# wenxiaoshuai/Points-Matching

Hardware: AMD Instinct MI355X
Metric: descriptor-pair distances/s (BF-L2 2-NN + ratio stage); RANSAC hypotheses/s in `ransac` (higher is better)
Workload: dtype f32

## Files before the change

### points_matching_amd/csrc/filter_gather.hip

```cpp
#include "pm_common.hpp"

namespace {

constexpr int FG_ROWS = 256;
constexpr int FG_MAX_BLOCKS = 4096;
constexpr unsigned FG_SPIN_LIMIT = 200000u;

enum { FG_RATIO = 0, FG_MIDPOINT = 1, FG_CROSS = 2 };
struct FgCross {
    const pm_match* rev;
    int nt, kr, flags;
};
struct FgParam {
    float ratio;
    double cut;
    FgCross x;
};

template <int MODE>
__device__ __forceinline__ bool fg_keep(const pm_match* __restrict__ knn, int i, int k, const FgParam& prm, pm_match& best)
{
    const uint4 a = *reinterpret_cast<const uint4*>(knn + static_cast<size_t>(i) * k);
    best.queryIdx = static_cast<int>(a.x); best.trainIdx = static_cast<int>(a.y);
    best.imgIdx = static_cast<int>(a.z);   best.distance = __uint_as_float(a.w);
// ... 141 lines not shown
template <int MODE>
__global__ __launch_bounds__(FG_ROWS) void filter_ratio_gather(const pm_match* __restrict__ knn, int nq, int k,
                                                               float ratio, const float* __restrict__ kp1,
                                                               const float* __restrict__ kp2,
                                                               pm_match* __restrict__ good, float* __restrict__ xy1,
                                                               float* __restrict__ xy2, int* __restrict__ n_out,
                                                               unsigned* __restrict__ blk_counts, unsigned epoch,
                                                               const unsigned long long* __restrict__ mm,
                                                               double* __restrict__ minmax_out)
{
    fg_compact<MODE>(knn, nq, k, ratio, kp1, kp2, good, xy1, xy2, n_out, blk_counts, epoch, mm, minmax_out,
                     FgCross{nullptr, 0, 0, 0});
}

__global__ __launch_bounds__(FG_ROWS) void filter_cross_gather(const pm_match* __restrict__ knn, int nq, int k, float ratio,
                                                               const float* __restrict__ kp1, const float* __restrict__ kp2,
                                                               pm_match* __restrict__ good, float* __restrict__ xy1,
                                                               float* __restrict__ xy2, int* __restrict__ n_out,
                                                               unsigned* __restrict__ blk_counts, unsigned epoch, FgCross cross)
{
    fg_compact<FG_CROSS>(knn, nq, k, ratio, kp1, kp2, good, xy1, xy2, n_out, blk_counts, epoch, nullptr, nullptr, cross);
}

__global__ __launch_bounds__(256) void concat_points(const float* __restrict__ xy1_parts,
                                                     const float* __restrict__ xy2_parts,
                                                     const int* __restrict__ counts, int parts, int stride,
                                                     float* __restrict__ xy1, float* __restrict__ xy2,
                                                     int* __restrict__ n_out)
{
    const int p = blockIdx.y;
    int off = 0, total = 0;
    for (int r = 0; r < parts; ++r) {
        int c = counts[r];
        c = c < 0 ? 0 : (c > stride ? stride : c);
        if (r < p) off += c;
        total += c;
    }
    int cp = counts[p];
    cp = cp < 0 ? 0 : (cp > stride ? stride : cp);
    const int i = blockIdx.x * 256 + threadIdx.x;
    if (i < cp) {
        const size_t s = 2 * (static_cast<size_t>(p) * stride + i), d = 2 * static_cast<size_t>(off + i);
        xy1[d] = xy1_parts[s]; xy1[d + 1] = xy1_parts[s + 1];
        xy2[d] = xy2_parts[s]; xy2[d + 1] = xy2_parts[s + 1];
    }
    if (p == 0 && i == 0) *n_out = total;
// ... 22 lines not shown

}

extern "C" int pm_filter_ratio_gather_dev(pm_ctx* ctx, const pm_match* d_knn, int nq, int k, float ratio,
                                          const float* d_kp1_xy, const float* d_kp2_xy, pm_match* d_good,
                                          float* d_xy1, float* d_xy2, int32_t* d_n_good)
{
    PM_REQUIRE(ctx != nullptr && d_n_good != nullptr, PM_E_INVALID, "null argument");
    PM_REQUIRE(nq >= 0 && k >= 2, PM_E_INVALID, "ratio test needs k >= 2");
    PM_REQUIRE(nq == 0 || (d_knn && d_good), PM_E_INVALID, "null match buffers");
    PM_REQUIRE((d_kp1_xy == nullptr) == (d_kp2_xy == nullptr), PM_E_INVALID, "give both keypoint arrays or none");
    PM_REQUIRE(d_kp1_xy == nullptr || (d_xy1 && d_xy2), PM_E_INVALID, "null point outputs");
    PM_HIP_CHECK(hipSetDevice(ctx->device));
    pm::ScopedKernelTime t(ctx, "filter_gather");
    if (nq == 0) {
        PM_HIP_CHECK(hipMemsetAsync(d_n_good, 0, sizeof(int32_t), ctx->stream));
        return PM_OK;
    }
    int nblk = 0;
    const int rc = fg_prepare(ctx, nq, &nblk);
    if (rc != PM_OK) return rc;
    hipLaunchKernelGGL(filter_ratio_gather<FG_RATIO>, dim3(nblk), dim3(FG_ROWS), 0, ctx->stream, d_knn, nq, k, ratio,
                       d_kp1_xy, d_kp2_xy, d_good, d_xy1, d_xy2, d_n_good, ctx->fg_counts, ctx->fg_epoch, nullptr, nullptr);
    PM_HIP_CHECK(hipGetLastError());
    return PM_OK;
}

extern "C" int pm_filter_midpoint_gather_dev(pm_ctx* ctx, const pm_match* d_m, int n, int k, const float* d_kp1_xy,
                                             const float* d_kp2_xy, pm_match* d_good, float* d_xy1, float* d_xy2,
                                             int32_t* d_n_good, double* d_minmax)
{
    PM_REQUIRE(ctx != nullptr && d_n_good != nullptr, PM_E_INVALID, "null argument");
    PM_REQUIRE(n >= 0 && k >= 1, PM_E_INVALID, "need n >= 0, k >= 1");
    PM_REQUIRE(n == 0 || (d_m && d_good), PM_E_INVALID, "null match buffers");
    PM_REQUIRE((d_kp1_xy == nullptr) == (d_kp2_xy == nullptr), PM_E_INVALID, "give both keypoint arrays or none");
    PM_REQUIRE(d_kp1_xy == nullptr || (d_xy1 && d_xy2), PM_E_INVALID, "null point outputs");
    PM_HIP_CHECK(hipSetDevice(ctx->device));
    pm::ScopedKernelTime t(ctx, "filter_gather");
    if (n == 0) {
        PM_HIP_CHECK(hipMemsetAsync(d_n_good, 0, sizeof(int32_t), ctx->stream));
        if (d_minmax) {
            const double init[2] = {1.0, 0.0};
            PM_HIP_CHECK(hipMemcpyAsync(d_minmax, init, sizeof init, hipMemcpyHostToDevice, ctx->stream));
            PM_HIP_CHECK(hipStreamSynchronize(ctx->stream));
        }
        return PM_OK;
// ... 58 lines not shown
```

### points_matching_amd/csrc/knn_constants.hpp

```cpp
#pragma once

namespace pm_knn {

constexpr int KNN_C = 4;
constexpr int QB = 128;
constexpr int TT32 = 64;
constexpr float KNN_BIG = 3.0e38f;

constexpr int H_DP = 128;
constexpr int H_ROW = H_DP + 16;
constexpr int H_LDS_ROW = H_ROW + 8;
constexpr int H_NCH = H_ROW / 16;
constexpr int H_TT = 128;
constexpr int H_QB = 256;
constexpr float H_MAXABS = 361.f;
constexpr int H_ROW16 = H_ROW / 8;
constexpr int H_LDS_ROW16 = H_LDS_ROW / 8;

constexpr int I8_BITS = 256;
constexpr int I8_NCH = 8;
constexpr int I8_ROW16 = 16;
constexpr int I8_LDS_ROW16 = 17;
constexpr int I8_GROUP_ROWS = 8;
constexpr int I8_SHIFT = 16;
constexpr int I8_EMPTY = static_cast<int>(0x80000000u);
constexpr int I8W_BITS = 512;
constexpr int I8W_NCH = 16;
constexpr int I8W_ROW16 = 32;

constexpr int U8_DP = 128;
constexpr int U8_NCH = 4;
constexpr int U8_ROW16 = 8;
constexpr int U8_LDS_ROW16 = 9;
constexpr int U8_SHIFT = 9;
constexpr int U8_PAD_SEED = -(1 << 22);
constexpr int U8_WIDE_ROW16 = 9;
constexpr int F16S_NCH = 8;
constexpr int F16S_ROW16 = 16;
constexpr int F16S_LDS_ROW16 = 17;
constexpr int SEED_TILE_BYTES = H_TT * 4;

}
```

### points_matching_amd/csrc/knn_l2.hip

```cpp
#include <cstdlib>

#include "knn_l2_plan.hpp"
#include "knn_shared.hpp"

namespace {

using namespace pm_knn;

constexpr int TILE_T = 64;
constexpr int PM_U8_FUSED_MAX_NQ = 768;
__host__ inline bool u8_fused_by_default(int nq) { return nq <= PM_U8_FUSED_MAX_NQ; }
constexpr float KNN_INF = __builtin_inff();

__device__ __forceinline__ uint32_t f32_bits(float f) { return __float_as_uint(f); }

__device__ __forceinline__ uint64_t knn_key(float dist, int idx)
{
    uint32_t b = (dist != dist) ? 0x7FC00000u : f32_bits(dist);
    return (static_cast<uint64_t>(b) << 32) | static_cast<uint32_t>(idx);
}

template <bool VEC4>
__device__ __forceinline__ float l2sqr_canonical(const float* __restrict__ a,
                                                 const float* __restrict__ b, int dim)
// ... 677 lines not shown
        const float t = a[j] - b[j];
        const float p = t * t;
        d = d + p;
    }
    return d;
}

struct KnnFuse {
    float ratio;
    const float* kp1;
    const float* kp2;
    pm_match* good;
    float* xy1;
    float* xy2;
    int* n_out;
    unsigned long long* pk;
    unsigned long long* tile;
    unsigned* tilecnt;
    unsigned* err;
    unsigned epoch;
};
constexpr int KF_TILE_BLOCKS = 8;
constexpr unsigned KF_SPIN_LIMIT = 1u << 22;

template <bool VEC4, int NS, bool FUSE, bool GEN, int KM>
__global__ __launch_bounds__(256) __attribute__((amdgpu_num_sgpr(80))) void knn_l2_refine(
    const float* __restrict__ Q, const float* __restrict__ T, const float* __restrict__ qnorm,
    const unsigned long long* __restrict__ stats, unsigned epoch, unsigned* __restrict__ diag, int nq, int nt,
    int dim, int k, KnnGeom g16, KnnGeom g32, int route, pm_match* __restrict__ out, KnnFuse fz)
{
    __shared__ int clist[4][64 * NS];
    const int lane = threadIdx.x & 63, wave = threadIdx.x >> 6;
    int q = __builtin_amdgcn_readfirstlane(blockIdx.x * 4 + wave);
    bool ghost = false;
    if (q >= nq) {
        if (!FUSE) return;
        ghost = true;
        q = nq - 1;
    }
    const float* qp = Q + static_cast<size_t>(q) * dim;
    const float na = qnorm[q];
    const unsigned long long s0 = stats[0], s1 = stats[1];
    const float tmax = static_cast<unsigned>(s0 >> 32) == epoch ? __uint_as_float(static_cast<unsigned>(s0)) : 0.f;
    const bool flagged = static_cast<unsigned>(s1 >> 32) == epoch;
    const bool ineligible = flagged && (s1 & 2ull);
    bool general = false;
    if constexpr (GEN) {
        const unsigned long long s3 = stats[3];
        const bool gen_off = static_cast<unsigned>(s3 >> 32) == epoch;
        general = route == ROUTE_AUTO && ineligible && !gen_off;
    }
    const bool hinted = route == ROUTE_F16_HINT || route == ROUTE_U8_HINT;
    const bool use16 = hinted || (route == ROUTE_AUTO && (!ineligible || general));
    const bool nonfinite = (flagged && (s1 & 1ull)) || (hinted && ineligible);
    const KnnGeom g = use16 ? g16 : g32;
    float unscale = 1.f, eps_c = g.eps_coef, eps_abs = 0.f;
    bool unranked = false;
    if constexpr (GEN) {
        if (general) {
// ... 98 lines not shown
    } else {
        for (int j = lane; j < nt; j += 64) {
            const float d =
                __builtin_sqrtf(l2sqr_canonical<VEC4>(qp, T + static_cast<size_t>(j) * dim, dim));
            b.insert(knn_key(d, j), d);
        }
    }
    int nn_idx[2] = {-1, -1};
    float nn_d[2] = {KNN_INF, KNN_INF};
    for (int c = 0; c < k; ++c) {
        const uint64_t best = wave_min_u64(b.k[0]);
        const unsigned long long owners = __ballot(b.k[0] == best);
        const int first = __ffsll(static_cast<long long>(owners)) - 1;
        const float dist = __shfl(b.d[0], first, 64);
        if (lane == first) b.pop();
        pm_match m;
        m.queryIdx = q;
        m.imgIdx = 0;
        if (best == ~0ull) { m.trainIdx = -1; m.distance = KNN_INF; }
        else { m.trainIdx = static_cast<int>(static_cast<uint32_t>(best)); m.distance = dist; }
        if (c < 2) { nn_idx[c] = m.trainIdx; nn_d[c] = m.distance; }
        if (lane == 0 && !ghost && out) out[static_cast<size_t>(q) * k + c] = m;
    }
    if (!FUSE) return;

    __shared__ unsigned s_keep[4];
    __shared__ unsigned s_bits;
    __shared__ int s_last;
    __shared__ int s_pre[4];
    const int tid = threadIdx.x;
    {
        const float rhs = fz.ratio * nn_d[1];
        const bool keep = !ghost && nn_idx[0] >= 0 && nn_idx[1] >= 0 && nn_d[0] < rhs;
        if (lane == 0) {
            if (!ghost)
                __hip_atomic_store(&fz.pk[q], (static_cast<unsigned long long>(f32_bits(nn_d[0])) << 32) |
                                                  static_cast<unsigned long long>(static_cast<uint32_t>(nn_idx[0])),
                                   __ATOMIC_RELAXED, __HIP_MEMORY_SCOPE_AGENT);
            s_keep[wave] = keep ? 1u : 0u;
        }
    }
    asm volatile("s_waitcnt vmcnt(0)" ::: "memory");
    __syncthreads();
    const int blk = static_cast<int>(blockIdx.x), tile = blk / KF_TILE_BLOCKS;
    const int nblk = static_cast<int>(gridDim.x), ntiles = (nblk + KF_TILE_BLOCKS - 1) / KF_TILE_BLOCKS;
    if (tid == 0) {
// ... 104 lines not shown
#pragma unroll
                for (int i = 0; i < U8_ROW16 / 2; ++i) tv[i] = tp[hf * (U8_ROW16 / 2) + i];
#pragma unroll
                for (int i = 0; i < U8_ROW16 / 2; ++i) {
                    const uint4 a = qv[hf * (U8_ROW16 / 2) + i];
                    acc = __builtin_amdgcn_sdot4(static_cast<int>(a.x), static_cast<int>(tv[i].x), acc, false);
                    acc = __builtin_amdgcn_sdot4(static_cast<int>(a.y), static_cast<int>(tv[i].y), acc, false);
                    acc = __builtin_amdgcn_sdot4(static_cast<int>(a.z), static_cast<int>(tv[i].z), acc, false);
                    acc = __builtin_amdgcn_sdot4(static_cast<int>(a.w), static_cast<int>(tv[i].w), acc, false);
                }
                asm volatile("" : "+v"(acc));
            }
            d2[u] = qn + static_cast<int>(tnorm[ok[u] ? row : row_begin]) - 2 * acc;
        }
#pragma unroll
        for (int u = 0; u < U; ++u) {
            const int row = base + u * LANES + me;
            const float d = __builtin_sqrtf(static_cast<float>(d2[u]));
            if (ok[u]) tb.insert(knn_key(d, row), d);
        }
    }
}

template <int NS, int GROUP, int KM, bool FUSE>
__global__ __launch_bounds__(256) void knn_l2_refine8(
    const float* __restrict__ Q, const float* __restrict__ T, const uint4* __restrict__ Q8, const uint4* __restrict__ T8,
    const float* __restrict__ qnorm, const float* __restrict__ tnorm, const int* __restrict__ cand,
    const unsigned long long* __restrict__ stats, unsigned epoch, unsigned* __restrict__ diag, int nq, int nt, int dim, int k,
    int slots, int tiles_per_split, pm_match* __restrict__ out, KnnFuse fz, int t_row16)
{
    constexpr int GPB = 16 / GROUP;
    constexpr int IMAX = 0x7FFFFFFF;
    __shared__ int clist[4][4][16 * NS];
    const int lane = threadIdx.x & 63, wave = threadIdx.x >> 6;
    const int qi = lane >> 4, l = lane & 15;
    const int q = blockIdx.x * 16 + wave * 4 + qi;
    const bool live = q < nq;
    const int qc = live ? q : nq - 1;
    const unsigned long long s1 = stats[1];
    const bool wrong_hint = static_cast<unsigned>(s1 >> 32) == epoch;
    if (diag && threadIdx.x == 0 && blockIdx.x == 0) diag[2] = 3u;
    const int qn = static_cast<int>(qnorm[qc]);
    const int* cv = cand + static_cast<size_t>(qc) * slots;
    uint4 qv[U8_ROW16];
#pragma unroll
    for (int i = 0; i < U8_ROW16; ++i) qv[i] = Q8[static_cast<size_t>(qc) * U8_ROW16 + i];

    int val[NS], code[NS];
    MinN<int, KM> mn;
    mn.init(IMAX);
#pragma unroll
    for (int i = 0; i < NS; ++i) {
        const int s = l + 16 * i;
// ... 97 lines not shown
            }
            for (int j = 0; j < KM; ++j) {
                const uint64_t m = pm::wave_min_u64(tb.k[0]);
                if (tb.k[0] == m && m != ~0ull) tb.pop();
                if (lane == src && m != ~0ull) b.insert(m, __uint_as_float(static_cast<unsigned>(m >> 32)));
            }
        }
    }
    int nn_idx[2] = {-1, -1};
    float nn_d[2] = {KNN_INF, KNN_INF};
    for (int c = 0; c < k; ++c) {
        const uint64_t best = row_min_u64(b.k[0]);
        const unsigned owners = static_cast<unsigned>(__ballot(b.k[0] == best) >> (16 * qi)) & 0xFFFFu;
        const int first = __ffs(static_cast<int>(owners)) - 1;
        const float dist = __shfl(b.d[0], 16 * qi + first, 64);
        if (l == first) b.pop();
        pm_match m;
        m.queryIdx = q;
        m.imgIdx = 0;
        if (best == ~0ull) { m.trainIdx = -1; m.distance = KNN_INF; }
        else { m.trainIdx = static_cast<int>(static_cast<uint32_t>(best)); m.distance = dist; }
        if (c < 2) { nn_idx[c] = m.trainIdx; nn_d[c] = m.distance; }
        if (l == 0 && live && out) out[static_cast<size_t>(q) * k + c] = m;
    }
    if constexpr (FUSE) {
        __shared__ unsigned s_bits[4];
        __shared__ unsigned long long s_rec[16];
        __shared__ int s_pre[4];
        const int tid = threadIdx.x;
        const float rhs = fz.ratio * nn_d[1];
        const bool keep = live && nn_idx[0] >= 0 && nn_idx[1] >= 0 && nn_d[0] < rhs;
        if (l == 0)
            s_rec[wave * 4 + qi] = (static_cast<unsigned long long>(f32_bits(nn_d[0])) << 32) |
                                   static_cast<unsigned long long>(static_cast<uint32_t>(nn_idx[0]));
        const unsigned long long bal = __ballot(l == 0 && keep);
        if (lane == 0)
            s_bits[wave] = static_cast<unsigned>(bal & 1ull) | (static_cast<unsigned>((bal >> 16) & 1ull) << 1) |
                           (static_cast<unsigned>((bal >> 32) & 1ull) << 2) | (static_cast<unsigned>((bal >> 48) & 1ull) << 3);
        __syncthreads();
        const unsigned bits = s_bits[0] | (s_bits[1] << 4) | (s_bits[2] << 8) | (s_bits[3] << 12);
        const int cnt = __popc(bits);
        const int blk = static_cast<int>(blockIdx.x);
        if (tid == 0)
            __hip_atomic_store(&fz.tilecnt[blk], (fz.epoch << 8) | static_cast<unsigned>(cnt), __ATOMIC_RELAXED, __HIP_MEMORY_SCOPE_AGENT);
        int before = 0;
        for (int j = tid; j < blk; j += 256) {
// ... 235 lines not shown
    const int tiles = (nq + queries_per_tile - 1) / queries_per_tile;
    if (tiles > ctx->kf_cap) {
        PM_HIP_CHECK(hipStreamSynchronize(ctx->stream));
        if (ctx->kf_tile) PM_HIP_CHECK(hipFree(ctx->kf_tile));
        ctx->kf_tile = nullptr;
        ctx->kf_cap = 0;
        const int cap = tiles < 4096 ? 4096 : tiles + tiles / 2;
        PM_HIP_CHECK(hipMalloc(reinterpret_cast<void**>(&ctx->kf_tile), static_cast<size_t>(cap) * 12));
        PM_HIP_CHECK(hipMemsetAsync(ctx->kf_tile, 0, static_cast<size_t>(cap) * 12, ctx->stream));
        ctx->kf_cap = cap;
        ctx->kf_epoch = 0;
    }
    if (++ctx->kf_epoch >= (1u << 24)) {
        PM_HIP_CHECK(hipMemsetAsync(ctx->kf_tile, 0, static_cast<size_t>(ctx->kf_cap) * 12, ctx->stream));
        ctx->kf_epoch = 1;
    }
    fz.tile = ctx->kf_tile;
    fz.tilecnt = reinterpret_cast<unsigned*>(ctx->kf_tile + ctx->kf_cap);
    fz.err = reinterpret_cast<unsigned*>(ctx->knn_stats) + 12;
    fz.epoch = ctx->kf_epoch;
    return PM_OK;
}

KnnL2Request knn_l2_request(const pm_ctx* ctx, const void* q, const void* t, bool u8_rows, int nq, int nt, int dim, int k, int flags,
                            bool fuse)
{
    KnnL2Request r{};
    r.nq = nq; r.nt = nt; r.dim = dim; r.k = k; r.flags = flags; r.n_cu = ctx->n_cu;
    std::memcpy(r.opts, ctx->opts, sizeof(r.opts));
    r.u8_rows = u8_rows;
    r.aligned = ((reinterpret_cast<uintptr_t>(q) | reinterpret_cast<uintptr_t>(t)) & (u8_rows ? 3 : 15)) == 0;
    r.fuse = fuse;
    return r;
}

KnnGeom knn_geom(const KnnGeomPlan& g, const float* cand)
{
    return KnnGeom{cand, g.slots, g.tiles_per_split, g.rows_per_tile, g.lid_mask, g.eps_coef, g.embed_coef, g.eps_coef_gen,
                   g.abs_gen, g.int_shift};
}

int knn_l2_enqueue(pm_ctx* ctx, const KnnL2Plan& p, const float* dq, int nq, const float* dt, int nt, int dim, int k,
                   pm_match* dout, const KnnFuse* fuse, const uint8_t* uq = nullptr, const uint8_t* ut = nullptr)
{
    PM_REFUSE_CAPTURE(ctx);
    int rc = pm::arena_reserve(ctx, p.need);
    if (rc != PM_OK) return rc;
    pm::arena_reset(ctx);
    float* qnorm = static_cast<float*>(pm::arena_take(ctx, p.qnorm_bytes));
    float* tnorm = static_cast<float*>(pm::arena_take(ctx, p.tnorm_bytes));
    float* cval32 = p.want32 ? static_cast<float*>(pm::arena_take(ctx, p.c32)) : nullptr;
    float* cval16 = p.want16 ? static_cast<float*>(pm::arena_take(ctx, p.c16)) : nullptr;
    _Float16* Qh = p.want16 ? static_cast<_Float16*>(pm::arena_take(ctx, p.qh)) : nullptr;
    _Float16* Th = p.want16 ? static_cast<_Float16*>(pm::arena_take(ctx, p.th)) : nullptr;
    void* seeds = p.sdb ? pm::arena_take(ctx, p.sdb) : nullptr;
    void* Qf = p.qfb ? pm::arena_take(ctx, p.qfb) : nullptr;
    PM_REQUIRE(qnorm && tnorm && (!p.want32 || cval32) && (!p.want16 || (cval16 && Qh && Th)) && (!p.sdb || seeds) && (!p.qfb || Qf),
               PM_E_NOMEM, "scratch arena too small");
    KnnFuse fz{};
    if (fuse) {
        fz = *fuse;
        fz.pk = static_cast<unsigned long long*>(pm::arena_take(ctx, p.pkb));
        PM_REQUIRE(fz.pk != nullptr, PM_E_NOMEM, "scratch arena too small");
        rc = kf_prepare(ctx, nq, fz, p.kf_tile);
        if (rc != PM_OK) return rc;
    }
    const KnnGeom g32 = knn_geom(p.g32, cval32), g16 = knn_geom(p.g16, cval16);

    unsigned long long* stats = ctx->knn_stats;
    if (++ctx->knn_epoch == 0u) {
        PM_HIP_CHECK(hipMemsetAsync(stats, 0, 32, ctx->stream));
        ctx->knn_epoch = 1u;
    }
    const unsigned epoch = ctx->knn_epoch;
    unsigned* diag = nullptr;
    if (ctx->knn_diag) {
        diag = ctx->knn_diag_words;
        PM_HIP_CHECK(hipMemsetAsync(diag, 0, 12, ctx->stream));
    }
    const int nq_pad = p.nq_pad, nt_pad = p.nt_pad, t_wide = p.t_wide, route = p.route;
    {
        pm::ScopedKernelTime t(ctx, "knn_l2_prep");
        const dim3 grid(p.prep_grid);
#define PM_PREP_DP_AL(LAUNCH_)                                                                                            \
    do {                                                                                                                  \
        if (p.dp16 == 128) { if (p.vec) LAUNCH_(128, true); else LAUNCH_(128, false); }                                   \
        else { if (p.vec) LAUNCH_(256, true); else LAUNCH_(256, false); }                                                 \
    } while (0)
#define PM_PREP16U(DP_, AL_)                                                                                              \
// ... 39 lines not shown
#undef PM_PREP_DP_AL
        PM_HIP_CHECK(hipGetLastError());
    }
    if (route == ROUTE_U8_HINT) {
        rc = launch_coarse_u8(ctx, Qh, Qf, Th, static_cast<const int*>(seeds), nq, nq_pad, nt, p.splits16, g16.tiles_per_split,
                              reinterpret_cast<int*>(cval16), g16.slots, p.u8_group, p.u8_form);
        if (rc != PM_OK) return rc;
    } else if (p.f16s) {
        rc = launch_coarse_f16s(ctx, Qh, Th, static_cast<const float*>(seeds), nq, nq_pad, nt, p.splits16, g16.tiles_per_split,
                                ~g16.lid_mask, cval16, g16.slots);
        if (rc != PM_OK) return rc;
    } else if (p.want16) {
        rc = launch_coarse_f16(ctx, Qh, Th, nq, nq_pad, nt, p.splits16, g16.tiles_per_split, ~g16.lid_mask, cval16,
                               g16.slots, stats, epoch, route == ROUTE_AUTO ? 1 : 0, p.dp16);
        if (rc != PM_OK) return rc;
    }
    if (p.want32) {
        rc = launch_coarse_f32(ctx, dq, nq, dt, nt, dim, tnorm, p.splits32, g32.tiles_per_split, ~g32.lid_mask, cval32,
                               g32.slots, stats, epoch, route == ROUTE_AUTO ? 1 : 0);
        if (rc != PM_OK) return rc;
    }
    pm::ScopedKernelTime t(ctx, "knn_l2_refine");
    if (p.refine8) {
#define PM_R8K(NS_, GROUP_, KM_, FUSE_)                                                                                    \
    hipLaunchKernelGGL((knn_l2_refine8<NS_, GROUP_, KM_, FUSE_>), dim3((nq + 15) / 16), dim3(256), 0, ctx->stream, dq, dt,  \
                       reinterpret_cast<const uint4*>(Qh), reinterpret_cast<const uint4*>(Th), qnorm, tnorm,               \
                       reinterpret_cast<const int*>(cval16), stats, epoch, diag, nq, nt, dim, k, g16.slots, g16.tiles_per_split, dout, fz, \
                       t_wide ? U8_WIDE_ROW16 : U8_ROW16)
#define PM_R8(NS_, GROUP_) do { if (p.refine_fuse) PM_R8K(NS_, GROUP_, 2, true); else if (p.refine_km == 2) PM_R8K(NS_, GROUP_, 2, false); else PM_R8K(NS_, GROUP_, 4, false); } while (0)
#define PM_R8G(NS_) do { if (p.refine_group == 4) PM_R8(NS_, 4); else if (p.refine_group == 8) PM_R8(NS_, 8); else PM_R8(NS_, 16); } while (0)
        switch (p.refine_ns) {
        case 1: PM_R8G(1); break;
        case 2: PM_R8G(2); break;
        case 4: PM_R8G(4); break;
        case 8: PM_R8G(8); break;
        default: PM_R8G(16); break;
        }
#undef PM_R8G
#undef PM_R8
#undef PM_R8K
    } else {
#define PM_REFINE5(VEC_, NS_, FUSE_, GEN_, KM_)                                                                      \
    hipLaunchKernelGGL((knn_l2_refine<VEC_, NS_, FUSE_, GEN_, KM_>), dim3((nq + 3) / 4), dim3(256), 0, ctx->stream, dq, dt,  \
                       qnorm, stats, epoch, diag, nq, nt, dim, k, g16, g32, route, dout, fz)
#define PM_REFINE4(VEC_, NS_, FUSE_, GEN_) do { if (p.refine_km == 2) PM_REFINE5(VEC_, NS_, FUSE_, GEN_, 2); else PM_REFINE5(VEC_, NS_, false, GEN_, 4); } while (0)
#define PM_REFINE3(NS_, FUSE_, GEN_) do { if (p.refine_vec) PM_REFINE4(true, NS_, FUSE_, GEN_); else PM_REFINE4(false, NS_, FUSE_, GEN_); } while (0)
#define PM_REFINE2(NS_, FUSE_) do { if (p.refine_gen) PM_REFINE3(NS_, FUSE_, true); else PM_REFINE3(NS_, FUSE_, false); } while (0)
#define PM_REFINE(NS_) do { if (p.refine_fuse) PM_REFINE2(NS_, true); else PM_REFINE2(NS_, false); } while (0)
        switch (p.refine_ns) {
        case 1: PM_REFINE(1); break;
        case 2: PM_REFINE(2); break;
        case 4: PM_REFINE(4); break;
        default: PM_REFINE(8); break;
        }
#undef PM_REFINE5
#undef PM_REFINE4
#undef PM_REFINE3
#undef PM_REFINE2
#undef PM_REFINE
    }
    PM_HIP_CHECK(hipGetLastError());
    return PM_OK;
}

int knn_l2_run(pm_ctx* ctx, const float* dq, int nq, const float* dt, int nt, int dim, int k, int flags, pm_match* dout,
               const KnnFuse* fuse, int* verdict, const uint8_t* uq = nullptr, const uint8_t* ut = nullptr)
{
    const bool u8 = uq != nullptr;
    const KnnL2Plan p = knn_l2_plan(knn_l2_request(ctx, u8 ? static_cast<const void*>(uq) : dq, u8 ? static_cast<const void*>(ut) : dt, u8,
                                                   nq, nt, dim, k, flags, fuse != nullptr));
    *verdict = p.verdict;
    if (p.verdict == KNN_EXACT) return run_exact(ctx, dq, nq, dt, nt, dim, k, dout);
    if (p.verdict == KNN_WIDEN) return PM_OK;
    return knn_l2_enqueue(ctx, p, dq, nq, dt, nt, dim, k, dout, fuse, uq, ut);
}

}

extern "C" int pm_bf_knn_l2_f32_dev(pm_ctx* ctx, const float* dq, int nq, const float* dt, int nt, int dim,
                                    int k, int flags, pm_match* dout)
{
    PM_REQUIRE(ctx != nullptr, PM_E_INVALID, "ctx is null");
    PM_REQUIRE(nq >= 0 && nt >= 0 && dim >= 1 && k >= 1 && k <= PM_MAX_K, PM_E_INVALID,
               "need nq,nt >= 0, dim >= 1, 1 <= k <= PM_MAX_K");
    PM_REQUIRE(nq == 0 || (dq && dout), PM_E_INVALID, "null query/output pointer");
    PM_REQUIRE(nt == 0 || dt, PM_E_INVALID, "null train pointer");
    if (nq == 0) return PM_OK;
    PM_HIP_CHECK(hipSetDevice(ctx->device));
    PM_REFUSE_CAPTURE(ctx);
    int verdict;
    return knn_l2_run(ctx, dq, nq, dt, nt, dim, k, flags, dout, nullptr, &verdict);
}

extern "C" int pm_bf_knn_l2_ratio_dev(pm_ctx* ctx, const float* d_q, int nq, const float* d_t, int nt, int dim, int flags,
                                      float ratio, const float* d_kp1_xy, const float* d_kp2_xy, pm_match* d_knn,
                                      pm_match* d_good, float* d_xy1, float* d_xy2, int32_t* d_n_good)
{
// ... 1 lines not shown
    PM_REQUIRE(nq >= 0 && nt >= 0 && dim >= 1, PM_E_INVALID, "need nq,nt >= 0, dim >= 1");
    PM_REQUIRE(nq == 0 || (d_q && d_good), PM_E_INVALID, "null query/output pointer");
    PM_REQUIRE(nt == 0 || d_t, PM_E_INVALID, "null train pointer");
    PM_REQUIRE((d_kp1_xy == nullptr) == (d_kp2_xy == nullptr), PM_E_INVALID, "give both keypoint arrays or none");
    PM_REQUIRE(d_kp1_xy == nullptr || (d_xy1 && d_xy2), PM_E_INVALID, "null point outputs");
    PM_HIP_CHECK(hipSetDevice(ctx->device));
    PM_REFUSE_CAPTURE(ctx);
    if (nq == 0) {
        PM_HIP_CHECK(hipMemsetAsync(d_n_good, 0, sizeof(int32_t), ctx->stream));
        return PM_OK;
    }
    KnnFuse fz{};
    fz.ratio = ratio; fz.kp1 = d_kp1_xy; fz.kp2 = d_kp2_xy; fz.good = d_good; fz.xy1 = d_xy1; fz.xy2 = d_xy2; fz.n_out = d_n_good;
    const int fusion = ctx->opts[PM_OPT_FILTER_FUSION];
    const bool u8_hint = (flags & PM_KNN_HINT_U8) && !(flags & (PM_KNN_FORCE_F32 | PM_KNN_FORCE_EXACT));
    const bool separate = fusion == 1 || (fusion == 0 && d_knn != nullptr && !(u8_hint && u8_fused_by_default(nq)));
    int rc, verdict;
    if (!separate) {
        rc = knn_l2_run(ctx, d_q, nq, d_t, nt, dim, 2, flags, d_knn, &fz, &verdict);
        if (rc != PM_OK || verdict == KNN_MATRIX) return rc;
        return pm_filter_ratio_gather_dev(ctx, d_knn, nq, 2, ratio, d_kp1_xy, d_kp2_xy, d_good, d_xy1, d_xy2, d_n_good);
    }
    PM_REQUIRE(d_knn != nullptr, PM_E_INVALID, "the two-launch form needs d_knn");
    rc = knn_l2_run(ctx, d_q, nq, d_t, nt, dim, 2, flags, d_knn, nullptr, &verdict);
    if (rc != PM_OK) return rc;
    return pm_filter_ratio_gather_dev(ctx, d_knn, nq, 2, ratio, d_kp1_xy, d_kp2_xy, d_good, d_xy1, d_xy2, d_n_good);
}

namespace {
int u8_widened(pm_ctx* ctx, const uint8_t* dq, int nq, const uint8_t* dt, int nt, int dim, const float** fq, const float** ft)
{
    const size_t a = pm::align_up(static_cast<size_t>(nq) * dim, 64), b = static_cast<size_t>(nt) * dim;
    if ((a + b) * sizeof(float) > ctx->widen_cap) {
        PM_HIP_CHECK(hipStreamSynchronize(ctx->stream));
        if (ctx->widen) PM_HIP_CHECK(hipFree(ctx->widen));
        ctx->widen = nullptr;
        ctx->widen_cap = 0;
        const size_t cap = pm::align_up((a + b) * sizeof(float) * 5 / 4, size_t(1) << 20);
        PM_HIP_CHECK(hipMalloc(reinterpret_cast<void**>(&ctx->widen), cap));
        ctx->widen_cap = cap;
    }
    if (static_cast<size_t>(nq) * dim)
        hipLaunchKernelGGL(knn_u8_widen, dim3(256), dim3(256), 0, ctx->stream, dq, static_cast<size_t>(nq) * dim, ctx->widen);
    if (b) hipLaunchKernelGGL(knn_u8_widen, dim3(256), dim3(256), 0, ctx->stream, dt, b, ctx->widen + a);
    PM_HIP_CHECK(hipGetLastError());
    *fq = ctx->widen;
    *ft = ctx->widen + a;
    return PM_OK;
// ... 22 lines not shown

extern "C" int pm_bf_knn_l2_u8_ratio_dev(pm_ctx* ctx, const uint8_t* d_q, int nq, const uint8_t* d_t, int nt, int dim, float ratio,
                                         const float* d_kp1_xy, const float* d_kp2_xy, pm_match* d_knn, pm_match* d_good,
                                         float* d_xy1, float* d_xy2, int32_t* d_n_good)
{
    PM_REQUIRE(ctx != nullptr && d_n_good != nullptr && d_knn != nullptr, PM_E_INVALID, "null argument (the u8 form needs the record buffer)");
    PM_REQUIRE(nq >= 0 && nt >= 0 && dim >= 1, PM_E_INVALID, "need nq,nt >= 0, dim >= 1");
    PM_REQUIRE(nq == 0 || (d_q && d_good), PM_E_INVALID, "null query/output pointer");
    PM_REQUIRE((d_kp1_xy == nullptr) == (d_kp2_xy == nullptr), PM_E_INVALID, "give both keypoint arrays or none");
    PM_REQUIRE(d_kp1_xy == nullptr || (d_xy1 && d_xy2), PM_E_INVALID, "null point outputs");
    PM_HIP_CHECK(hipSetDevice(ctx->device));
    PM_REFUSE_CAPTURE(ctx);
    if (nq == 0) {
        PM_HIP_CHECK(hipMemsetAsync(d_n_good, 0, sizeof(int32_t), ctx->stream));
        return PM_OK;
    }
    const int fusion = ctx->opts[PM_OPT_FILTER_FUSION];
    if (fusion == 2 || (fusion == 0 && u8_fused_by_default(nq))) {
        KnnFuse fz{};
        fz.ratio = ratio; fz.kp1 = d_kp1_xy; fz.kp2 = d_kp2_xy; fz.good = d_good; fz.xy1 = d_xy1; fz.xy2 = d_xy2; fz.n_out = d_n_good;
        int verdict;
        const int rf = knn_l2_run(ctx, nullptr, nq, nullptr, nt, dim, 2, 0, d_knn, &fz, &verdict, d_q, d_t);
        if (rf != PM_OK || verdict != KNN_WIDEN) return rf;
    }
    const int rc = pm_bf_knn_l2_u8_dev(ctx, d_q, nq, d_t, nt, dim, 2, d_knn);
    if (rc != PM_OK) return rc;
    return pm_filter_ratio_gather_dev(ctx, d_knn, nq, 2, ratio, d_kp1_xy, d_kp2_xy, d_good, d_xy1, d_xy2, d_n_good);
}

extern "C" int pm_bf_knn_l2_u8(pm_ctx* ctx, const uint8_t* q, int nq, const uint8_t* t, int nt, int dim, int k, pm_match* out)
{
    PM_REQUIRE(ctx != nullptr, PM_E_INVALID, "ctx is null");
    PM_REQUIRE(nq >= 0 && nt >= 0 && dim >= 1 && k >= 1 && k <= PM_MAX_K, PM_E_INVALID,
               "need nq,nt >= 0, dim >= 1, 1 <= k <= PM_MAX_K");
    PM_REQUIRE(nq == 0 || (q && out), PM_E_INVALID, "null query/output pointer");
    PM_REQUIRE(nt == 0 || t, PM_E_INVALID, "null train pointer");
    if (nq == 0) return PM_OK;
    PM_HIP_CHECK(hipSetDevice(ctx->device));
    return pm::StagedBlock::knn(ctx, __func__, q, static_cast<size_t>(nq) * dim, t, static_cast<size_t>(nt) * dim, out,
                                  sizeof(pm_match) * static_cast<size_t>(nq) * k, [&](void* dq, void* dt, void* dout) {
        return pm_bf_knn_l2_u8_dev(ctx, static_cast<const uint8_t*>(dq), nq, static_cast<const uint8_t*>(dt), nt, dim, k,
                                   static_cast<pm_match*>(dout));
    });
}

extern "C" int pm_bf_knn_l2_f32(pm_ctx* ctx, const float* q, int nq, const float* t, int nt, int dim, int k,
// ... 16 lines not shown
```

### points_matching_amd/csrc/pm_capi.cpp

```cpp
#include <cfloat>
#include <cmath>

#include "pm_common.hpp"

namespace pm {

static thread_local char g_err[512] = "";

void set_error(const char* fmt, ...)
{
    va_list ap;
    va_start(ap, fmt);
    vsnprintf(g_err, sizeof g_err, fmt, ap);
    va_end(ap);
}

int arena_reserve(pm_ctx* ctx, size_t bytes)
{
    if (bytes <= ctx->arena_cap) return PM_OK;
    PM_HIP_CHECK(hipStreamSynchronize(ctx->stream));
    if (ctx->arena) PM_HIP_CHECK(hipFree(ctx->arena));
    ctx->arena = nullptr;
    ctx->arena_cap = 0;
    size_t cap = align_up(bytes + bytes / 4, size_t(1) << 20);
// ... 154 lines not shown
    if (e != hipSuccess) {
        set_error("hipMalloc failed: %s", hipGetErrorString(e));
        (void)hipStreamDestroy(c->own_stream);
        delete c;
        return PM_E_NOMEM;
    }
    c->knn_diag_words = reinterpret_cast<unsigned*>(c->knn_stats + 4);
    *out = c;
    return PM_OK;
}

int pm_ctx_destroy(pm_ctx* ctx)
{
    if (!ctx) return PM_OK;
    (void)hipSetDevice(ctx->device);
    (void)hipStreamSynchronize(ctx->stream);
    drain_timers(ctx);
    for (hipEvent_t e : ctx->event_pool) (void)hipEventDestroy(e);
    if (ctx->arena) (void)hipFree(ctx->arena);
    if (ctx->knn_stats) (void)hipFree(ctx->knn_stats);
    if (ctx->fg_counts) (void)hipFree(ctx->fg_counts);
    if (ctx->sync_words) (void)hipFree(ctx->sync_words);
    if (ctx->kf_tile) (void)hipFree(ctx->kf_tile);
    if (ctx->widen) (void)hipFree(ctx->widen);
    if (ctx->feat) (void)hipFree(ctx->feat);
    if (ctx->desc_tab) (void)hipFree(ctx->desc_tab);
    if (ctx->pinned) (void)hipHostFree(ctx->pinned);
    if (ctx->own_stream) (void)hipStreamDestroy(ctx->own_stream);
    delete ctx;
    return PM_OK;
}

int pm_ctx_set_stream(pm_ctx* ctx, void* hip_stream)
{
    PM_REQUIRE(ctx != nullptr, PM_E_INVALID, "ctx is null");
    PM_HIP_CHECK(hipStreamSynchronize(ctx->stream));
    ctx->stream = hip_stream ? static_cast<hipStream_t>(hip_stream) : ctx->own_stream;
    return PM_OK;
}

int pm_ctx_synchronize(pm_ctx* ctx)
{
    PM_REQUIRE(ctx != nullptr, PM_E_INVALID, "ctx is null");
    PM_HIP_CHECK(hipStreamSynchronize(ctx->stream));
    return PM_OK;
}
// ... 330 lines not shown
```

### points_matching_amd/csrc/pm_common.hpp

```cpp
#pragma once
#include <hip/hip_runtime.h>

#include <cstdarg>
#include <cstdint>
#include <cstdio>
#include <cstring>
#include <map>
#include <string>
#include <vector>

#include "pm.h"
#include "stage_layout.hpp"

namespace pm {

void set_error(const char* fmt, ...);

#define PM_HIP_CHECK(expr)                                                              \
    do {                                                                                \
        hipError_t e_ = (expr);                                                         \
        if (e_ != hipSuccess) {                                                         \
            ::pm::set_error("%s failed: %s (%s:%d)", #expr, hipGetErrorString(e_),      \
                            __FILE__, __LINE__);                                        \
            return PM_E_HIP;                                                            \
// ... 29 lines not shown

struct pm_ctx {
    int device = 0;
    hipStream_t own_stream = nullptr;
    hipStream_t stream = nullptr;
    char* arena = nullptr;
    size_t arena_cap = 0;
    size_t arena_off = 0;
    void* pinned = nullptr;
    size_t pinned_cap = 0;
    bool timing = false;
    std::map<std::string, pm::KernelTimer> timers;
    std::vector<hipEvent_t> event_pool;
    int n_cu = 256;
    unsigned long long* knn_stats = nullptr;
    unsigned* knn_diag_words = nullptr;
    unsigned knn_epoch = 0;
    bool knn_diag = false;
    unsigned* fg_counts = nullptr;
    unsigned fg_epoch = 0;
    unsigned long long* kf_tile = nullptr;
    int kf_cap = 0;
    unsigned kf_epoch = 0;
    int* sync_words = nullptr;
    int opts[PM_OPT_COUNT_] = {};
    float* widen = nullptr;
    size_t widen_cap = 0;
    char* feat = nullptr;
    size_t feat_cap = 0;
    size_t feat_counter_off = 0;
    int feat_noct = 0;
    int feat_w[16] = {}, feat_h[16] = {};
    size_t feat_off[16] = {};
    char* desc_tab = nullptr;
};

namespace pm {

int arena_reserve(pm_ctx* ctx, size_t bytes);
void arena_reset(pm_ctx* ctx);
void* arena_take(pm_ctx* ctx, size_t bytes);
int pinned_reserve(pm_ctx* ctx, size_t bytes);
struct __attribute__((visibility("hidden"))) StagedBlock : StageLayout {
    pm_ctx* ctx;
    const char* who;
    char* base = nullptr;
    int rc = PM_OK;
    StagedBlock(pm_ctx* c, const char* w) : ctx(c), who(w) {}
    StagedBlock(const StagedBlock&) = delete;
    ~StagedBlock();
    int alloc();
    void upload(size_t off, const void* src, size_t bytes);
    void download(void* dst, size_t off, size_t bytes);
    int sync();
    template <class T> T* at(size_t off) const { return reinterpret_cast<T*>(base + off); }
    void step(hipError_t e, int status, const char* what);
    template <class Dev> static int knn(pm_ctx* ctx, const char* who, const void* q, size_t qb, const void* t, size_t tb, void* out, size_t ob, Dev dev)
    {
        StagedBlock bq(ctx, who), bt(ctx, who), bo(ctx, who);
        const size_t o_q = bq.add(qb), o_t = bt.add(tb), o_out = bo.add(ob);
        if (bq.alloc() != PM_OK || bt.alloc() != PM_OK || bo.alloc() != PM_OK) return PM_E_NOMEM;
        bq.upload(o_q, q, qb);
        if (bq.rc == PM_OK) bt.upload(o_t, t, tb);
        if (bq.rc != PM_OK || bt.rc != PM_OK) return PM_E_HIP;
        bo.rc = dev(bq.base, bt.base, bo.base);
// ... 58 lines not shown
```

Measured before the change: 2272 billion.

## Emit ratio-test keep masks from refine kernel and compact via mask prefix sums

In the two-launch, non-fused k=2 path, the refine kernel now evaluates the ratio test itself and writes one keep bit per query into a small mask buffer. A new compaction kernel reads those masks and computes global offsets by having each block popcount all preceding mask words. This replaces the ratio-filter kernel's cross-block counter handshake with spin waits and its re-evaluation of the test. The cost is a redundant O(blocks²) popcount over mask words, a new device mask buffer, and an extra template variant for the refine kernels.

```diff
diff --git a/points_matching_amd/csrc/filter_gather.hip b/points_matching_amd/csrc/filter_gather.hip
--- a/points_matching_amd/csrc/filter_gather.hip
+++ b/points_matching_amd/csrc/filter_gather.hip
@@ -1,3 +1,4 @@
+#include "knn_constants.hpp"
 #include "pm_common.hpp"
 
 namespace {
@@ -187,6 +188,60 @@
     fg_compact<FG_CROSS>(knn, nq, k, ratio, kp1, kp2, good, xy1, xy2, n_out, blk_counts, epoch, nullptr, nullptr, cross);
 }
 
+__global__ __launch_bounds__(FG_ROWS) void filter_masks_kernel(const uint4* __restrict__ masks, const pm_match* __restrict__ knn,
+                                                               int nq, int k, const float* __restrict__ kp1,
+                                                               const float* __restrict__ kp2, pm_match* __restrict__ good,
+                                                               float* __restrict__ xy1, float* __restrict__ xy2,
+                                                               int* __restrict__ n_out)
+{
+    __shared__ int wave_cnt[FG_ROWS / 64];
+    __shared__ int wave_pre[FG_ROWS / 64];
+    const int tid = threadIdx.x, lane = tid & 63, wave = tid >> 6;
+    const int b = blockIdx.x;
+    const int i = b * FG_ROWS + tid;
+    constexpr int V16 = FG_ROWS / 64;
+    const int ic = i < nq ? i : nq - 1;
+    const uint4 a = *reinterpret_cast<const uint4*>(knn + static_cast<size_t>(ic) * k);
+    const uint4 own = masks[b * V16 + wave];
+    float2 pa = {0.f, 0.f}, pb = {0.f, 0.f};
+    if (kp1) pa = *reinterpret_cast<const float2*>(kp1 + 2 * static_cast<size_t>(ic));
+    int before = 0;
+    for (int v = tid; v < b * V16; v += FG_ROWS) {
+        const uint4 m = masks[v];
+        before += __popc(m.x) + __popc(m.y) + __popc(m.z) + __popc(m.w);
+    }
+    if (kp1) {
+        const int tr = static_cast<int>(a.y);
+        pb = *reinterpret_cast<const float2*>(kp2 + 2 * static_cast<size_t>(tr >= 0 ? tr : 0));
+    }
+    const unsigned ow = (lane >> 4) == 0 ? own.x : (lane >> 4) == 1 ? own.y : (lane >> 4) == 2 ? own.z : own.w;
+    const bool keep = i < nq && ((ow >> (8 * ((lane >> 2) & 3) + (lane & 3))) & 1u);
+#pragma unroll
+    for (int o = 32; o > 0; o >>= 1) before += __shfl_xor(before, o, 64);
+    const unsigned long long bal = __ballot(keep);
+    if (lane == 0) { wave_cnt[wave] = __popcll(bal); wave_pre[wave] = before; }
+    __syncthreads();
+    int off = __popcll(bal & ((1ull << lane) - 1ull));
+    int tot = 0;
+#pragma unroll
+    for (int w = 0; w < FG_ROWS / 64; ++w) {
+        off += wave_pre[w];
+        if (w < wave) off += wave_cnt[w];
+        tot += wave_pre[w] + wave_cnt[w];
+    }
+    if (keep) {
+        pm_match best;
+        best.queryIdx = static_cast<int>(a.x); best.trainIdx = static_cast<int>(a.y);
+        best.imgIdx = static_cast<int>(a.z);   best.distance = __uint_as_float(a.w);
+        good[off] = best;
+        if (kp1) {
+            *reinterpret_cast<float2*>(xy1 + 2 * static_cast<size_t>(off)) = pa;
+            *reinterpret_cast<float2*>(xy2 + 2 * static_cast<size_t>(off)) = pb;
+        }
+    }
+    if (b == static_cast<int>(gridDim.x) - 1 && tid == 0) *n_out = tot;
+}
+
 __global__ __launch_bounds__(256) void concat_points(const float* __restrict__ xy1_parts,
                                                      const float* __restrict__ xy2_parts,
                                                      const int* __restrict__ counts, int parts, int stride,
@@ -255,6 +310,22 @@
     if (rc != PM_OK) return rc;
     hipLaunchKernelGGL(filter_ratio_gather<FG_RATIO>, dim3(nblk), dim3(FG_ROWS), 0, ctx->stream, d_knn, nq, k, ratio,
                        d_kp1_xy, d_kp2_xy, d_good, d_xy1, d_xy2, d_n_good, ctx->fg_counts, ctx->fg_epoch, nullptr, nullptr);
+    PM_HIP_CHECK(hipGetLastError());
+    return PM_OK;
+}
+
+static_assert(FG_ROWS == pm_knn::KM_BLOCK_ROWS && FG_MAX_BLOCKS * FG_ROWS == pm_knn::KM_MAX_ROWS,
+              "the mask buffer is sized in this compaction's blocks");
+
+int pm::filter_masks_gather(pm_ctx* ctx, const pm_match* d_knn, int nq, int k, const float* d_kp1_xy, const float* d_kp2_xy,
+                            pm_match* d_good, float* d_xy1, float* d_xy2, int32_t* d_n_good)
+{
+    const int nblk = (nq + FG_ROWS - 1) / FG_ROWS;
+    PM_REQUIRE(nq >= 1 && nblk <= FG_MAX_BLOCKS, PM_E_UNSUPPORTED, "more than 1M query rows per compaction call");
+    PM_REQUIRE(ctx->km_masks != nullptr && pm_knn::knn_mask_bytes(nq) <= ctx->km_cap, PM_E_INVALID, "no keep masks for this many rows");
+    pm::ScopedKernelTime t(ctx, "filter_gather");
+    hipLaunchKernelGGL(filter_masks_kernel, dim3(nblk), dim3(FG_ROWS), 0, ctx->stream, reinterpret_cast<const uint4*>(ctx->km_masks),
+                       d_knn, nq, k, d_kp1_xy, d_kp2_xy, d_good, d_xy1, d_xy2, d_n_good);
     PM_HIP_CHECK(hipGetLastError());
     return PM_OK;
 }
diff --git a/points_matching_amd/csrc/knn_constants.hpp b/points_matching_amd/csrc/knn_constants.hpp
--- a/points_matching_amd/csrc/knn_constants.hpp
+++ b/points_matching_amd/csrc/knn_constants.hpp
@@ -1,4 +1,5 @@
 #pragma once
+#include <cstddef>
 
 namespace pm_knn {
 
@@ -40,4 +41,17 @@
 constexpr int F16S_LDS_ROW16 = 17;
 constexpr int SEED_TILE_BYTES = H_TT * 4;
 
+constexpr int KM_BLOCK_ROWS = 256;
+constexpr int KM_BLOCK_BYTES = KM_BLOCK_ROWS / 4;
+constexpr int KM_MAX_ROWS = 4096 * KM_BLOCK_ROWS;
+inline size_t knn_mask_bytes(int nq)
+{
+    return (static_cast<size_t>(nq) + KM_BLOCK_ROWS - 1) / KM_BLOCK_ROWS * KM_BLOCK_BYTES;
 }
+inline size_t knn_mask_capacity(size_t need)
+{
+    const size_t want = need + need / 2;
+    return want < 4096 ? 4096 : (want + KM_BLOCK_BYTES - 1) / KM_BLOCK_BYTES * KM_BLOCK_BYTES;
+}
+
+}
diff --git a/points_matching_amd/csrc/knn_l2.hip b/points_matching_amd/csrc/knn_l2.hip
--- a/points_matching_amd/csrc/knn_l2.hip
+++ b/points_matching_amd/csrc/knn_l2.hip
@@ -723,19 +723,21 @@
 };
 constexpr int KF_TILE_BLOCKS = 8;
 constexpr unsigned KF_SPIN_LIMIT = 1u << 22;
-
-template <bool VEC4, int NS, bool FUSE, bool GEN, int KM>
+enum { KNN_TAIL_NONE = 0, KNN_TAIL_FUSE = 1, KNN_TAIL_MASK = 2 };
+
+template <bool VEC4, int NS, int TAIL, bool GEN, int KM>
 __global__ __launch_bounds__(256) __attribute__((amdgpu_num_sgpr(80))) void knn_l2_refine(
     const float* __restrict__ Q, const float* __restrict__ T, const float* __restrict__ qnorm,
     const unsigned long long* __restrict__ stats, unsigned epoch, unsigned* __restrict__ diag, int nq, int nt,
-    int dim, int k, KnnGeom g16, KnnGeom g32, int route, pm_match* __restrict__ out, KnnFuse fz)
-{
+    int dim, int k, KnnGeom g16, KnnGeom g32, int route, pm_match* __restrict__ out, KnnFuse fz, uint8_t* __restrict__ masks)
+{
+    constexpr bool FUSE = TAIL == KNN_TAIL_FUSE;
     __shared__ int clist[4][64 * NS];
     const int lane = threadIdx.x & 63, wave = threadIdx.x >> 6;
     int q = __builtin_amdgcn_readfirstlane(blockIdx.x * 4 + wave);
     bool ghost = false;
     if (q >= nq) {
-        if (!FUSE) return;
+        if (TAIL == KNN_TAIL_NONE) return;
         ghost = true;
         q = nq - 1;
     }
@@ -880,6 +882,14 @@
         if (c < 2) { nn_idx[c] = m.trainIdx; nn_d[c] = m.distance; }
         if (lane == 0 && !ghost && out) out[static_cast<size_t>(q) * k + c] = m;
     }
+    if constexpr (TAIL == KNN_TAIL_MASK) {
+        __shared__ unsigned s_bit[4];
+        const float rhs = fz.ratio * nn_d[1];
+        const bool keep = !ghost && nn_idx[0] >= 0 && nn_idx[1] >= 0 && nn_d[0] < rhs;
+        if (lane == 0) s_bit[wave] = keep ? 1u << wave : 0u;
+        __syncthreads();
+        if (threadIdx.x == 0) masks[blockIdx.x] = static_cast<uint8_t>(s_bit[0] | s_bit[1] | s_bit[2] | s_bit[3]);
+    }
     if (!FUSE) return;
 
     __shared__ unsigned s_keep[4];
@@ -1030,13 +1040,14 @@
     }
 }
 
-template <int NS, int GROUP, int KM, bool FUSE>
+template <int NS, int GROUP, int KM, int TAIL>
 __global__ __launch_bounds__(256) void knn_l2_refine8(
     const float* __restrict__ Q, const float* __restrict__ T, const uint4* __restrict__ Q8, const uint4* __restrict__ T8,
     const float* __restrict__ qnorm, const float* __restrict__ tnorm, const int* __restrict__ cand,
     const unsigned long long* __restrict__ stats, unsigned epoch, unsigned* __restrict__ diag, int nq, int nt, int dim, int k,
-    int slots, int tiles_per_split, pm_match* __restrict__ out, KnnFuse fz, int t_row16)
-{
+    int slots, int tiles_per_split, pm_match* __restrict__ out, KnnFuse fz, uint8_t* __restrict__ masks, int t_row16)
+{
+    constexpr bool FUSE = TAIL == KNN_TAIL_FUSE;
     constexpr int GPB = 16 / GROUP;
     constexpr int IMAX = 0x7FFFFFFF;
     __shared__ int clist[4][4][16 * NS];
@@ -1180,6 +1191,14 @@
         else { m.trainIdx = static_cast<int>(static_cast<uint32_t>(best)); m.distance = dist; }
         if (c < 2) { nn_idx[c] = m.trainIdx; nn_d[c] = m.distance; }
         if (l == 0 && live && out) out[static_cast<size_t>(q) * k + c] = m;
+    }
+    if constexpr (TAIL == KNN_TAIL_MASK) {
+        const float rhs = fz.ratio * nn_d[1];
+        const bool keep = live && nn_idx[0] >= 0 && nn_idx[1] >= 0 && nn_d[0] < rhs;
+        const unsigned long long bal = __ballot(l == 0 && keep);
+        if (lane == 0)
+            masks[blockIdx.x * 4 + wave] = static_cast<uint8_t>((bal & 1ull) | (((bal >> 16) & 1ull) << 1) |
+                                                                (((bal >> 32) & 1ull) << 2) | (((bal >> 48) & 1ull) << 3));
     }
     if constexpr (FUSE) {
         __shared__ unsigned s_bits[4];
@@ -1461,6 +1480,21 @@
     return PM_OK;
 }
 
+int km_prepare(pm_ctx* ctx, int nq)
+{
+    const size_t need = knn_mask_bytes(nq);
+    if (need > ctx->km_cap) {
+        PM_HIP_CHECK(hipStreamSynchronize(ctx->stream));
+        if (ctx->km_masks) PM_HIP_CHECK(hipFree(ctx->km_masks));
+        ctx->km_masks = nullptr;
+        ctx->km_cap = 0;
+        const size_t cap = knn_mask_capacity(need);
+        PM_HIP_CHECK(hipMalloc(reinterpret_cast<void**>(&ctx->km_masks), cap));
+        ctx->km_cap = cap;
+    }
+    return PM_OK;
+}
+
 KnnL2Request knn_l2_request(const pm_ctx* ctx, const void* q, const void* t, bool u8_rows, int nq, int nt, int dim, int k, int flags,
                             bool fuse)
 {
@@ -1480,7 +1514,8 @@
 }
 
 int knn_l2_enqueue(pm_ctx* ctx, const KnnL2Plan& p, const float* dq, int nq, const float* dt, int nt, int dim, int k,
-                   pm_match* dout, const KnnFuse* fuse, const uint8_t* uq = nullptr, const uint8_t* ut = nullptr)
+                   pm_match* dout, const KnnFuse* fuse, const uint8_t* uq = nullptr, const uint8_t* ut = nullptr,
+                   const float* mask_ratio = nullptr)
 {
     PM_REFUSE_CAPTURE(ctx);
     int rc = pm::arena_reserve(ctx, p.need);
@@ -1504,6 +1539,14 @@
         rc = kf_prepare(ctx, nq, fz, p.kf_tile);
         if (rc != PM_OK) return rc;
     }
+    const bool mask_tail = mask_ratio != nullptr && !p.refine_fuse && p.refine_km == 2;
+    PM_REQUIRE(mask_ratio == nullptr || mask_tail, PM_E_INVALID, "the mask tail needs a k = 2 plan without the fused tail");
+    if (mask_tail) {
+        fz.ratio = *mask_ratio;
+        rc = km_prepare(ctx, nq);
+        if (rc != PM_OK) return rc;
+    }
+    uint8_t* masks = mask_tail ? ctx->km_masks : nullptr;
     const KnnGeom g32 = knn_geom(p.g32, cval32), g16 = knn_geom(p.g16, cval16);
 
     unsigned long long* stats = ctx->knn_stats;
@@ -1589,12 +1632,12 @@
     }
     pm::ScopedKernelTime t(ctx, "knn_l2_refine");
     if (p.refine8) {
-#define PM_R8K(NS_, GROUP_, KM_, FUSE_)                                                                                    \
-    hipLaunchKernelGGL((knn_l2_refine8<NS_, GROUP_, KM_, FUSE_>), dim3((nq + 15) / 16), dim3(256), 0, ctx->stream, dq, dt,  \
+#define PM_R8K(NS_, GROUP_, KM_, TAIL_)                                                                                    \
+    hipLaunchKernelGGL((knn_l2_refine8<NS_, GROUP_, KM_, TAIL_>), dim3((nq + 15) / 16), dim3(256), 0, ctx->stream, dq, dt,  \
                        reinterpret_cast<const uint4*>(Qh), reinterpret_cast<const uint4*>(Th), qnorm, tnorm,               \
                        reinterpret_cast<const int*>(cval16), stats, epoch, diag, nq, nt, dim, k, g16.slots, g16.tiles_per_split, dout, fz, \
-                       t_wide ? U8_WIDE_ROW16 : U8_ROW16)
-#define PM_R8(NS_, GROUP_) do { if (p.refine_fuse) PM_R8K(NS_, GROUP_, 2, true); else if (p.refine_km == 2) PM_R8K(NS_, GROUP_, 2, false); else PM_R8K(NS_, GROUP_, 4, false); } while (0)
+                       masks, t_wide ? U8_WIDE_ROW16 : U8_ROW16)
+#define PM_R8(NS_, GROUP_) do { if (p.refine_fuse) PM_R8K(NS_, GROUP_, 2, KNN_TAIL_FUSE); else if (mask_tail) PM_R8K(NS_, GROUP_, 2, KNN_TAIL_MASK); else if (p.refine_km == 2) PM_R8K(NS_, GROUP_, 2, KNN_TAIL_NONE); else PM_R8K(NS_, GROUP_, 4, KNN_TAIL_NONE); } while (0)
 #define PM_R8G(NS_) do { if (p.refine_group == 4) PM_R8(NS_, 4); else if (p.refine_group == 8) PM_R8(NS_, 8); else PM_R8(NS_, 16); } while (0)
         switch (p.refine_ns) {
         case 1: PM_R8G(1); break;
@@ -1607,13 +1650,13 @@
 #undef PM_R8
 #undef PM_R8K
     } else {
-#define PM_REFINE5(VEC_, NS_, FUSE_, GEN_, KM_)                                                                      \
-    hipLaunchKernelGGL((knn_l2_refine<VEC_, NS_, FUSE_, GEN_, KM_>), dim3((nq + 3) / 4), dim3(256), 0, ctx->stream, dq, dt,  \
-                       qnorm, stats, epoch, diag, nq, nt, dim, k, g16, g32, route, dout, fz)
-#define PM_REFINE4(VEC_, NS_, FUSE_, GEN_) do { if (p.refine_km == 2) PM_REFINE5(VEC_, NS_, FUSE_, GEN_, 2); else PM_REFINE5(VEC_, NS_, false, GEN_, 4); } while (0)
-#define PM_REFINE3(NS_, FUSE_, GEN_) do { if (p.refine_vec) PM_REFINE4(true, NS_, FUSE_, GEN_); else PM_REFINE4(false, NS_, FUSE_, GEN_); } while (0)
-#define PM_REFINE2(NS_, FUSE_) do { if (p.refine_gen) PM_REFINE3(NS_, FUSE_, true); else PM_REFINE3(NS_, FUSE_, false); } while (0)
-#define PM_REFINE(NS_) do { if (p.refine_fuse) PM_REFINE2(NS_, true); else PM_REFINE2(NS_, false); } while (0)
+#define PM_REFINE5(VEC_, NS_, TAIL_, GEN_, KM_)                                                                      \
+    hipLaunchKernelGGL((knn_l2_refine<VEC_, NS_, TAIL_, GEN_, KM_>), dim3((nq + 3) / 4), dim3(256), 0, ctx->stream, dq, dt,  \
+                       qnorm, stats, epoch, diag, nq, nt, dim, k, g16, g32, route, dout, fz, masks)
+#define PM_REFINE4(VEC_, NS_, TAIL_, GEN_) do { if (p.refine_km == 2) PM_REFINE5(VEC_, NS_, TAIL_, GEN_, 2); else PM_REFINE5(VEC_, NS_, KNN_TAIL_NONE, GEN_, 4); } while (0)
+#define PM_REFINE3(NS_, TAIL_, GEN_) do { if (p.refine_vec) PM_REFINE4(true, NS_, TAIL_, GEN_); else PM_REFINE4(false, NS_, TAIL_, GEN_); } while (0)
+#define PM_REFINE2(NS_, TAIL_) do { if (p.refine_gen) PM_REFINE3(NS_, TAIL_, true); else PM_REFINE3(NS_, TAIL_, false); } while (0)
+#define PM_REFINE(NS_) do { if (p.refine_fuse) PM_REFINE2(NS_, KNN_TAIL_FUSE); else if (mask_tail) PM_REFINE2(NS_, KNN_TAIL_MASK); else PM_REFINE2(NS_, KNN_TAIL_NONE); } while (0)
         switch (p.refine_ns) {
         case 1: PM_REFINE(1); break;
         case 2: PM_REFINE(2); break;
@@ -1631,7 +1674,8 @@
 }
 
 int knn_l2_run(pm_ctx* ctx, const float* dq, int nq, const float* dt, int nt, int dim, int k, int flags, pm_match* dout,
-               const KnnFuse* fuse, int* verdict, const uint8_t* uq = nullptr, const uint8_t* ut = nullptr)
+               const KnnFuse* fuse, int* verdict, const uint8_t* uq = nullptr, const uint8_t* ut = nullptr,
+               const float* mask_ratio = nullptr)
 {
     const bool u8 = uq != nullptr;
     const KnnL2Plan p = knn_l2_plan(knn_l2_request(ctx, u8 ? static_cast<const void*>(uq) : dq, u8 ? static_cast<const void*>(ut) : dt, u8,
@@ -1639,7 +1683,7 @@
     *verdict = p.verdict;
     if (p.verdict == KNN_EXACT) return run_exact(ctx, dq, nq, dt, nt, dim, k, dout);
     if (p.verdict == KNN_WIDEN) return PM_OK;
-    return knn_l2_enqueue(ctx, p, dq, nq, dt, nt, dim, k, dout, fuse, uq, ut);
+    return knn_l2_enqueue(ctx, p, dq, nq, dt, nt, dim, k, dout, fuse, uq, ut, mask_ratio);
 }
 
 }
@@ -1687,8 +1731,11 @@
         return pm_filter_ratio_gather_dev(ctx, d_knn, nq, 2, ratio, d_kp1_xy, d_kp2_xy, d_good, d_xy1, d_xy2, d_n_good);
     }
     PM_REQUIRE(d_knn != nullptr, PM_E_INVALID, "the two-launch form needs d_knn");
-    rc = knn_l2_run(ctx, d_q, nq, d_t, nt, dim, 2, flags, d_knn, nullptr, &verdict);
+    const bool masked = fusion == 0 && nq <= KM_MAX_ROWS;
+    rc = knn_l2_run(ctx, d_q, nq, d_t, nt, dim, 2, flags, d_knn, nullptr, &verdict, nullptr, nullptr, masked ? &ratio : nullptr);
     if (rc != PM_OK) return rc;
+    if (masked && verdict == KNN_MATRIX)
+        return pm::filter_masks_gather(ctx, d_knn, nq, 2, d_kp1_xy, d_kp2_xy, d_good, d_xy1, d_xy2, d_n_good);
     return pm_filter_ratio_gather_dev(ctx, d_knn, nq, 2, ratio, d_kp1_xy, d_kp2_xy, d_good, d_xy1, d_xy2, d_n_good);
 }
 
@@ -1757,6 +1804,12 @@
         int verdict;
         const int rf = knn_l2_run(ctx, nullptr, nq, nullptr, nt, dim, 2, 0, d_knn, &fz, &verdict, d_q, d_t);
         if (rf != PM_OK || verdict != KNN_WIDEN) return rf;
+    } else if (fusion == 0 && nq <= KM_MAX_ROWS) {
+        int verdict;
+        const int rm = knn_l2_run(ctx, nullptr, nq, nullptr, nt, dim, 2, 0, d_knn, nullptr, &verdict, d_q, d_t, &ratio);
+        if (rm != PM_OK) return rm;
+        if (verdict == KNN_MATRIX)
+            return pm::filter_masks_gather(ctx, d_knn, nq, 2, d_kp1_xy, d_kp2_xy, d_good, d_xy1, d_xy2, d_n_good);
     }
     const int rc = pm_bf_knn_l2_u8_dev(ctx, d_q, nq, d_t, nt, dim, 2, d_knn);
     if (rc != PM_OK) return rc;
diff --git a/points_matching_amd/csrc/pm_capi.cpp b/points_matching_amd/csrc/pm_capi.cpp
--- a/points_matching_amd/csrc/pm_capi.cpp
+++ b/points_matching_amd/csrc/pm_capi.cpp
@@ -200,6 +200,7 @@
     if (ctx->fg_counts) (void)hipFree(ctx->fg_counts);
     if (ctx->sync_words) (void)hipFree(ctx->sync_words);
     if (ctx->kf_tile) (void)hipFree(ctx->kf_tile);
+    if (ctx->km_masks) (void)hipFree(ctx->km_masks);
     if (ctx->widen) (void)hipFree(ctx->widen);
     if (ctx->feat) (void)hipFree(ctx->feat);
     if (ctx->desc_tab) (void)hipFree(ctx->desc_tab);
diff --git a/points_matching_amd/csrc/pm_common.hpp b/points_matching_amd/csrc/pm_common.hpp
--- a/points_matching_amd/csrc/pm_common.hpp
+++ b/points_matching_amd/csrc/pm_common.hpp
@@ -75,6 +75,8 @@
     unsigned long long* kf_tile = nullptr;
     int kf_cap = 0;
     unsigned kf_epoch = 0;
+    uint8_t* km_masks = nullptr;
+    size_t km_cap = 0;
     int* sync_words = nullptr;
     int opts[PM_OPT_COUNT_] = {};
     float* widen = nullptr;
@@ -94,6 +96,9 @@
 void arena_reset(pm_ctx* ctx);
 void* arena_take(pm_ctx* ctx, size_t bytes);
 int pinned_reserve(pm_ctx* ctx, size_t bytes);
+__attribute__((visibility("hidden"))) int filter_masks_gather(pm_ctx* ctx, const pm_match* d_knn, int nq, int k, const float* d_kp1_xy,
+                                                              const float* d_kp2_xy, pm_match* d_good, float* d_xy1, float* d_xy2,
+                                                              int32_t* d_n_good);
 struct __attribute__((visibility("hidden"))) StagedBlock : StageLayout {
     pm_ctx* ctx;
     const char* who;
```

Result: faster. 2308 billion, median of 5 (+1.6%).
